# TimingSpace/MVOScaleRecovery

Hardware: AMD Instinct MI355X
Metric: frames/sec scale-recovery, KITTI-00 flow (~2k feats/frame), 1/2/4/8 GPU (higher is better)
Workload: dtype f64

## Files before the change

mvoscalerecovery_amd/csrc/mvosr_kernels.hip:

```cpp
#include <hip/hip_runtime.h>
#include <math.h>
#include <stdint.h>
#include <stdlib.h>
#include <string.h>

#include "../../include/mvosr.h"
#include "mvosr_device.hpp"
#include "mvosr_host.hpp"

namespace mvosr {

#ifdef MVOSR_STAMPS
#define MVOSR_STAMP(i) do { if (threadIdx.x == 0 && stamps) stamps[i] = __builtin_amdgcn_s_memtime(); } while (0)
#define MVOSR_STAMP_DECL unsigned long long stamps[12] = {0,0,0,0,0,0,0,0,0,0,0,0};
#define MVOSR_STAMP_ARG , unsigned long long *stamps = nullptr
#define MVOSR_STAMP_PASS , stamps
#define MVOSR_RSTAMP(i) do { if (stamps) stamps[i] = __builtin_amdgcn_s_memtime(); } while (0)
#else
#define MVOSR_RSTAMP(i) do {} while (0)
#define MVOSR_STAMP(i) do {} while (0)
#define MVOSR_STAMP_DECL
#define MVOSR_STAMP_ARG
#define MVOSR_STAMP_PASS
#endif
// ... 15 lines not shown
    p.misc = p.red + 8u * (uint32_t)(kRedSlots * 2 * waves);
    p.total = p.misc + 4u * 32u;
    return p;
}

struct Smem {
    double2 *P;
    double *Y;
    uint16_t *c16;
    uint32_t *c32;
    uint32_t *sel;
    int *hist;
    double *red;
    int *misc;
};
__device__ __forceinline__ Smem carve(char *base, int n, int waves) {
    const LdsPlan p = lds_plan(n, waves);
    Smem s;
    s.P = reinterpret_cast<double2 *>(base + p.p);
    s.Y = reinterpret_cast<double *>(base + p.y);
    s.c16 = reinterpret_cast<uint16_t *>(base + p.c);
    s.c32 = reinterpret_cast<uint32_t *>(base + p.c);
    s.sel = reinterpret_cast<uint32_t *>(base + p.c);
    s.hist = reinterpret_cast<int *>(base + p.hist);
    s.red = reinterpret_cast<double *>(base + p.red);
    s.misc = reinterpret_cast<int *>(base + p.misc);
    return s;
}

enum { M_WCNT = 0 , M_LIST = 16, M_MEDLO = 18, M_MEDHI = 20  };


constexpr int kTC = 2;


typedef double dvec2 __attribute__((ext_vector_type(2)));
__device__ __forceinline__ double2 stream_load2(const double2 *p) {
    const dvec2 v = __builtin_nontemporal_load(reinterpret_cast<const dvec2 *>(p));
    double2 r; r.x = v.x; r.y = v.y;
    return r;
}
__device__ __forceinline__ double stream_load(const double *p) {
    return __builtin_nontemporal_load(p);
}

template <int B>
struct TriChunk {
    TriIds q[kTC];
    template <bool STREAM = false>
    __device__ __forceinline__ void load(const int32_t *tri, int64_t begin, int count, int base, int tid) {
#pragma unroll
        for (int k = 0; k < kTC; ++k) {
            const int t = base + k * B + tid;
            if (t < count) {
                if constexpr (STREAM) {
                    const int32_t *p = tri + 3 * begin + 3 * t;
                    q[k].a = __builtin_nontemporal_load(p); q[k].b = __builtin_nontemporal_load(p + 1); q[k].c = __builtin_nontemporal_load(p + 2);
                } else {
                    q[k] = load_tri(tri + 3 * begin, t);
                }
            }
        }
    }
};

struct VoteFlags { bool f0, f1, f2; };
// ... 232 lines not shown
    pitch = asin(-uy) * 180.0 / 3.141592653589793;
    if (pitch < thr_deg) r |= 1;
    if (pitch >= thr_deg) r |= 2;
    return r;
}
__device__ __attribute__((noinline)) int pitch_reference_cold(double x0, double y0, double z0, double x1, double y1, double z1,
                                                              double x2, double y2, double z2, double thr_deg) {
    double nx, ny, nz, pitch;
    return pitch_reference_impl<false>(x0, y0, z0, x1, y1, z1, x2, y2, z2, thr_deg, nx, ny, nz, pitch);
}
template <bool FULL>
__device__ __forceinline__ int pitch_reference(double x0, double y0, double z0, double x1, double y1, double z1,
                                               double x2, double y2, double z2, double thr_deg,
                                               double &nx, double &ny, double &nz, double &pitch) {
    if constexpr (FULL) return pitch_reference_impl<true>(x0, y0, z0, x1, y1, z1, x2, y2, z2, thr_deg, nx, ny, nz, pitch);
    else { nx = ny = nz = pitch = 0.0; return pitch_reference_cold(x0, y0, z0, x1, y1, z1, x2, y2, z2, thr_deg); }
}

struct SelectResult {
    double height_level;
    int n_pitch, n_tri_valid;
    int singular, bad;
    int n_steep;
    int near;
};

enum { MODE_HOT = 0, MODE_EXACT = 1, MODE_FULL = 2 };

struct PitchTest {
    double thr_deg;
    double s2_hi, s2_lo;
};

template <bool FULL>
__device__ __forceinline__ int classify_triangle(double x0, double y0, double z0, double x1, double y1, double z1,
                                                 double x2, double y2, double z2, double h, const PitchTest &pt,
                                                 double *g_normals, double *g_pitch, double *g_heights, int64_t tg) {
    bool is_flat = false, is_steep = false, is_singular = false;
    bool decided = false;
    if constexpr (!FULL) {
        const double e1x = x1 - x0, e1y = y1 - y0, e1z = z1 - z0;
        const double e2x = x2 - x0, e2y = y2 - y0, e2z = z2 - z0;
        const double cx = __builtin_fma(e1y, e2z, -(e1z * e2y));
        const double cy = __builtin_fma(e1z, e2x, -(e1x * e2z));
        const double cz = __builtin_fma(e1x, e2y, -(e1y * e2x));
        const double tx = x0 * cx, ty = y0 * cy, tz = z0 * cz;
        const double det = (tx + ty) + tz;
        const double mag = (fabs(tx) + fabs(ty)) + fabs(tz);
        const double c2 = __builtin_fma(cz, cz, __builtin_fma(cy, cy, cx * cx));
        const double q2 = cy * cy;
        const double sy = cy * det;
        const bool safe = fabs(det) > 1e-9 * mag;
        is_flat = safe & (sy > 0.0) & (q2 > pt.s2_hi * c2);
        is_steep = safe & ((sy <= 0.0) | (q2 < pt.s2_lo * c2));
        decided = is_flat | is_steep;
    }
    if (!decided) {
        double nx, ny, nz, pitch;
        const int r = pitch_reference<FULL>(x0, y0, z0, x1, y1, z1, x2, y2, z2, pt.thr_deg, nx, ny, nz, pitch);
        is_singular = r & 4;
        is_flat = r & 1;
        is_steep = r & 2;
        if constexpr (FULL) {
            if (g_normals) { double *o = g_normals + 3 * tg; o[0] = nx; o[1] = ny; o[2] = nz; }
            if (g_pitch) g_pitch[tg] = pitch;
            if (g_heights) g_heights[tg] = h;
        }
    }
    return (is_flat ? 1 : 0) | (is_steep ? 2 : 0) | (is_singular ? 4 : 0) | (decided ? 0 : 8);
}

template <bool FULL, class Fetch>
struct SteepStream {
    const int32_t *tri;
    const int32_t *order;
    int t2n;
    const PitchTest &pt;
    Fetch fetch;
    int t_next;
    unsigned long long mask;
    double h;
    __device__ __forceinline__ void refill() {
        const int t = t_next + lane_id();
        bool steep = false;
        h = 0.0;
        if (t < t2n) {
            const int row = order ? min(max(order[t], 0), t2n - 1) : t;
            const TriIds q = load_tri(tri, row);
            double x0, y0, z0, x1, y1, z1, x2, y2, z2;
            if (fetch(q, x0, y0, z0, x1, y1, z1, x2, y2, z2)) {
// ... 81 lines not shown
        });
        __threadfence_block();
        __syncthreads();
        if (tid == 0) {
            double val[kNpDepth + 1];
            int vp = 0, kk = 0;
            np_pairwise_leaves(m, [&](int, int, bool is_leaf) {
                if (is_leaf) val[vp++] = leaf[kk++];
                else { const double r = val[--vp], l = val[--vp]; val[vp++] = l + r; }
            });
            *slot = c0 == 0 ? val[0] : *slot + val[0];
        }
        __syncthreads();
    }
    res = *slot;
    __syncthreads();
    return (0.0 + res) / (double)n_steep;
}

struct LdsFetch {
    const double2 *P; const double *Y; int n_valid;
    __device__ __forceinline__ bool operator()(const TriIds q, double &x0, double &y0, double &z0, double &x1, double &y1, double &z1,
                                               double &x2, double &y2, double &z2) const {
        if ((unsigned)q.a >= (unsigned)n_valid || (unsigned)q.b >= (unsigned)n_valid || (unsigned)q.c >= (unsigned)n_valid) return false;
        const double2 p0 = P[q.a], p1 = P[q.b], p2 = P[q.c];
        x0 = p0.x; z0 = p0.y; x1 = p1.x; z1 = p1.y; x2 = p2.x; z2 = p2.y;
        y0 = Y[q.a]; y1 = Y[q.b]; y2 = Y[q.c];
        return true;
    }
};

constexpr double kLevelGuard = 1e-12;

template <int WAVES, int MODE, int FW = 1>
__device__ __forceinline__ SelectResult phase_select(const Smem &s, int n_valid, const int32_t *tri2, int64_t t2_begin,
                                                     int t2_count, TriChunk<WAVES * kWave> &tc, PitchTest pt,
                                                     double *g_normals, double *g_pitch, double *g_heights, int bad_in,
                                                     double *scratch, int scratch_cap MVOSR_STAMP_ARG) {
    constexpr int B = WAVES * kWave;
    constexpr bool FULL = MODE == MODE_FULL;
    const int tid = threadIdx.x;
    unsigned long long flat = 0ull;
    unsigned long long flat_hi = 0ull;
    double hsum = 0.0, hcnt = 0.0, habs = 0.0;
    int npitch = 0, singular = 0, bad = 0;
    int undecided = 0;
    if (t2_count > 64 * FW * B) { bad = 1; t2_count = 0; }
    auto test_triangle = [&](int t, int kk, const TriIds q) {
    if ((unsigned)q.a >= (unsigned)n_valid || (unsigned)q.b >= (unsigned)n_valid || (unsigned)q.c >= (unsigned)n_valid) { bad = 1; return; }
    const double2 p0 = s.P[q.a], p1 = s.P[q.b], p2 = s.P[q.c];
    const double y0 = s.Y[q.a], y1 = s.Y[q.b], y2 = s.Y[q.c];
    const double x0 = p0.x, z0 = p0.y, x1 = p1.x, z1 = p1.y, x2 = p2.x, z2 = p2.y;
    const double h = MODE == MODE_HOT ? (y0 + y1) + y2 : div3((y0 + y1) + y2);
    const int r = classify_triangle<FULL>(x0, y0, z0, x1, y1, z1, x2, y2, z2, h, pt, g_normals, g_pitch, g_heights, t2_begin + t);
    const bool is_flat = r & 1, is_steep = r & 2;
    if (r & 4) singular = 1;
    if constexpr (MODE == MODE_HOT) { if (r & 8) undecided = 1; }
    if (is_steep) { hsum += h; hcnt += 1.0; if constexpr (MODE == MODE_HOT) habs += fabs(h); }
    if (is_flat) {
        if (FW == 1 || kk < 64) flat |= 1ull << (kk & 63); else flat_hi |= 1ull << (kk & 63);
        ++npitch;
    }
    };
    TriChunk<B> tn;
    for (int base = 0; base < t2_count; base += kTC * B) {
        const bool more = base + kTC * B < t2_count;
        if (more) tn.load(tri2, t2_begin, t2_count, base + kTC * B, tid);
#pragma unroll
        for (int k = 0; k < kTC; ++k) {
            const int t = base + k * B + tid;
            if (t < t2_count) test_triangle(t, base / B + k, tc.q[k]);
        }
        if (more) tc = tn;
    }
    const bool in_regs = t2_count <= kTC * B;
    if (!in_regs && t2_count > 0) tc.template load<true>(tri2, t2_begin, t2_count, 0, tid);
    if constexpr (MODE == MODE_HOT) block_sum3<WAVES>(hsum, hcnt, habs, s.red + R_SEL_H * 2 * WAVES, s.red + R_SEL_ABS * 2 * WAVES);
    else block_sum2<WAVES>(hsum, hcnt, s.red + R_SEL_H * 2 * WAVES);
    MVOSR_STAMP(4);
    SelectResult r;
    double hl = hsum / hcnt;
    const double guard = kLevelGuard * (habs / hcnt);
    if constexpr (MODE != MODE_HOT) {
        if (scratch && (int)hcnt + kNpMaxLeaves <= scratch_cap)
            hl = exact_height_level_block<WAVES, FULL>(tri2 + 3 * t2_begin, t2_count, (int)hcnt, pt, LdsFetch{s.P, s.Y, n_valid}, nullptr,
                                                       scratch, s.misc + M_WCNT, s.red + R_MISC * 2 * WAVES);
        else
            hl = exact_height_level<FULL>(tri2 + 3 * t2_begin, t2_count, (int)hcnt, pt, LdsFetch{s.P, s.Y, n_valid});
    }
    int ntv = 0, near = undecided;
    auto mark_triangle = [&](int kk, int qa, int qb, int qc) {
        const unsigned long long fw = (FW == 1 || kk < 64) ? flat : flat_hi;
        if (!((fw >> (kk & 63)) & 1ull)) return;
        const double y0 = s.Y[qa], y1 = s.Y[qb], y2 = s.Y[qc];
        const double h = MODE == MODE_HOT ? (y0 + y1) + y2 : div3((y0 + y1) + y2);
        if constexpr (MODE == MODE_HOT) { if (fabs(h - hl) <= guard) near = 1; }
        if (h > hl) {
            ++ntv;
            atomicOr(&s.sel[qa >> 5], 1u << (qa & 31));
            atomicOr(&s.sel[qb >> 5], 1u << (qb & 31));
            atomicOr(&s.sel[qc >> 5], 1u << (qc & 31));
        }
    };
    for (int base = 0; base < t2_count; base += kTC * B) {
        const bool more = base + kTC * B < t2_count;
        if (more) tn.template load<true>(tri2, t2_begin, t2_count, base + kTC * B, tid);
#pragma unroll
        for (int k = 0; k < kTC; ++k) {
            if (base + k * B + tid < t2_count) mark_triangle(base / B + k, tc.q[k].a, tc.q[k].b, tc.q[k].c);
        }
        if (more) tc = tn;
    }
    bad |= bad_in;
    int sn = singular | (near << 16);
    block_sum4i<WAVES>(npitch, ntv, sn, bad, s.red + R_SEL_CNT * 2 * WAVES);
    singular = sn & 0xFFFF;
    r.near = sn >> 16;
    MVOSR_STAMP(5);
    r.height_level = MODE == MODE_HOT ? hl / 3.0 : hl;
    r.n_steep = (int)hcnt;
    r.n_pitch = npitch; r.n_tri_valid = ntv; r.singular = singular; r.bad = bad;
    return r;
}

struct RoadResult {
    double height;
    int status;
    int n_sel, n_kept, n_modes, mode_left, mode_right;
    double mean, std, skew, median;
};

__device__ __forceinline__ bool dropped_by_single(double y, int bin, const Bits192 &single, int first_single) {
    bool d = false;
#pragma unroll
    for (int dk = -1; dk <= 1; ++dk) {
        const int k = bin + dk;
        const bool is_single = (k >= 0) && (k < kBins) && single.test_lane(max(k, 0));
// ... 401 lines not shown
    int32_t *c = a.o.counts + f * MVOSR_N_COUNTS;
    c[MVOSR_CNT_VALID] = nvalid; c[MVOSR_CNT_TRI_PITCH] = npitch; c[MVOSR_CNT_TRI_VALID] = ntv;
    c[MVOSR_CNT_SELECTED] = R.n_sel; c[MVOSR_CNT_KEPT] = R.n_kept; c[MVOSR_CNT_MODES] = R.n_modes;
    c[MVOSR_CNT_MODE_LEFT] = R.mode_left; c[MVOSR_CNT_MODE_RIGHT] = R.mode_right;
}

__device__ __forceinline__ bool early_frame_exit(const KArgs &a, int64_t f, int n, int t2n) {
    const bool too_few = n == 3;
    const bool oversize = n > a.b.max_feat;
    if (!(n <= 2 || too_few || t2n <= 0 || oversize)) return false;
    if (threadIdx.x == 0) {
        RoadResult R;
        R.n_sel = R.n_kept = R.n_modes = 0; R.mode_left = R.mode_right = -1;
        a.o.raw_scale[f] = nan(""); a.o.height[f] = nan(""); a.o.height_level[f] = nan("");
        a.o.status[f] = oversize ? MVOSR_ST_ERR_MASK : (too_few ? MVOSR_ST_TOO_FEW : MVOSR_ST_ERR_EMPTY);
        a.nsel[f] = 0;
        write_counts(a, f, too_few ? n : 0, 0, 0, R);
    }
    return true;
}

template <int BW, int MODE>
__device__ __forceinline__ void frame_tail(const KArgs &a, const Smem &s, int64_t f, int64_t off, int nvalid, bool refused,
                                           SelectResult &S, RoadResult &R) {
    constexpr int B = BW * kWave;
    const int tid = threadIdx.x;
    int status = kStPending;
    double raw = nan("");
    int nsel = 0;
    if (refused || S.bad) {
        status = MVOSR_ST_ERR_MASK;
    } else if (S.singular) {
        status = MVOSR_ST_ERR_SINGULAR;
    } else {
        const int w = wave_id(), lane = lane_id();
        const int per = ((nvalid + B - 1) / B) * kWave;
        const int begin = w * per, end = min(nvalid, begin + per);
        int cnt = 0;
        for (int j0 = begin; j0 < end; j0 += kWave) {
            const int j = j0 + lane;
            const bool sel = (j < end) && ((s.sel[j >> 5] >> (j & 31)) & 1u);
            if (a.o.selected && j < end) a.o.selected[off + j] = (uint8_t)sel;
            cnt += __popcll(__ballot(sel));
        }
        if (lane == 0) s.misc[M_WCNT + w] = cnt;
        __syncthreads();
        int base = 0;
#pragma unroll
        for (int i = 0; i < BW; ++i) { const int c = s.misc[M_WCNT + i]; if (i < w) base += c; nsel += c; }
        if constexpr (MODE == MODE_HOT) {
            if (S.near || nsel == 0) {
                if (tid == 0) { a.redo[1 + atomicAdd(a.redo, 1)] = (int32_t)f; a.o.status[f] = kStRedo; a.nsel[f] = 0; }
                return;
            }
        }
        double *dst = a.ysel + off;
        for (int j0 = begin; j0 < end; j0 += kWave) {
            const int j = j0 + lane;
            const bool sel = (j < end) && ((s.sel[j >> 5] >> (j & 31)) & 1u);
            const unsigned long long m = __ballot(sel);
            if (sel) dst[base + __popcll(m & ((1ull << lane) - 1ull))] = s.Y[j];
            base += __popcll(m);
        }
        if (nsel == 0) { status = MVOSR_ST_NO_FLAT; raw = a.P.absolute_reference / S.height_level; }
    }
    if (tid == 0) {
// ... 35 lines not shown
    MVOSR_STAMP_DECL
    MVOSR_STAMP(11);
    const int n = a.b.feat_cnt[f];
    const int64_t off = a.b.feat_off[f];
    const int64_t t1b = a.b.tri1_off[f], t2b = a.b.tri2_off[f];
    const int t1n = tri_rows(a.b.tri1_off, a.b.tri1_cnt, f), t2n = tri_rows(a.b.tri2_off, a.b.tri2_cnt, f);
    const Smem s = carve(smem, n, WAVES);
#ifdef MVOSR_STAMPS
    if (n < 0) return;
#endif
    MVOSR_STAMP(0);
#ifdef MVOSR_STAMPS
    if (threadIdx.x == 0) {
        stamps[10] = (unsigned long long)__builtin_amdgcn_s_getreg((31 << 11) | 4) | ((unsigned long long)__builtin_amdgcn_s_getreg((31 << 11) | 20) << 32);
    }
#endif

    RoadResult R;
    R.height = nan(""); R.n_sel = R.n_kept = R.n_modes = 0; R.mode_left = R.mode_right = -1;
    R.mean = R.std = R.skew = R.median = nan("");
    if (early_frame_exit(a, f, n, t2n)) return;
    int bad = 0;
    TriChunk<B> tc2;
    const int nvalid = phase_vote<WAVES, SC>(s, n, a.b.x + off, a.b.y + off, a.b.z + off, a.b.v + off, a.b.tri1, t1b, t1n,
                                             a.P.cos_pitch, a.P.sin_pitch,
                                             a.o.vote_counters ? a.o.vote_counters + off : nullptr, bad,
                                             a.b.tri2, t2b, t2n, tc2, a.P.vote_mode == MVOSR_VOTE_FIXED MVOSR_STAMP_PASS);
    const bool mask_mismatch = a.b.n2_expected && a.b.n2_expected[f] != nvalid;

    SelectResult S;
    S.height_level = nan(""); S.n_pitch = S.n_tri_valid = 0; S.singular = 0; S.bad = 1; S.n_steep = 0; S.near = 0;
    const bool too_many_rows = t1n > kMaxVoteRows;
    if (!mask_mismatch && !too_many_rows)
        S = phase_select<WAVES, MODE>(s, nvalid, a.b.tri2, t2b, t2n, tc2, a.pt, a.o.tri_normals, a.o.tri_pitch_deg,
                                      a.o.tri_heights, bad, a.ysel ? a.ysel + off : nullptr, n MVOSR_STAMP_PASS);
    frame_tail<WAVES, MODE>(a, s, f, off, nvalid, mask_mismatch || too_many_rows, S, R);
    MVOSR_STAMP(9);
#ifdef MVOSR_STAMPS
    if (threadIdx.x == 0 && a.o.hist) { unsigned long long *d = reinterpret_cast<unsigned long long *>(a.o.hist + f * 2 * kBins); for (int i = 0; i < 12; ++i) d[i] = stamps[i]; }
#endif
    });
}

struct DenseWs { double2 *P2; double *Y2; };

__host__ __device__ inline uint32_t dense_lds_bytes(int n, int waves) {
    const uint32_t npad = (uint32_t)((n + 1) & ~1);
    return align16(2u * npad + 16u) + align16(4u * ((uint32_t)(n + 31) / 32u)) + 8u * (uint32_t)(kRedSlots * 2 * waves) + 4u * 32u;
}

template <int DW, bool FUSED>
__device__ __forceinline__ int phase_vote_dense(uint32_t *c32, int *misc, int n, const double *gx, const double *gy, const double *gz,
                                                const double *gv, const int32_t *tri1, int64_t t1_begin, int t1_count,
                                                double cp, double sp, int32_t *g_counters, int &bad,
                                                double2 *P2, double *Y2, bool fixed) {
    constexpr int B = DW * kWave;
    const int tid = threadIdx.x, w = wave_id(), lane = lane_id();
    const uint16_t *c16 = reinterpret_cast<const uint16_t *>(c32);
    const uint32_t ones = ((uint32_t)(kCounterBias + 1) << 16) | (uint32_t)(kCounterBias + 1);
    for (int i = tid; i < ((n + 1) >> 1); i += B) c32[i] = ones;
    __threadfence_block();
    __syncthreads();
    const bool checked = t1_count > kMaxVoteRows;
    for (int t = tid; t < t1_count; t += B) {
        const TriIds q = load_tri(tri1 + 3 * t1_begin, t);
        if ((unsigned)q.a >= (unsigned)n || (unsigned)q.b >= (unsigned)n || (unsigned)q.c >= (unsigned)n) { bad = 1; continue; }
        double2 p0, p1, p2;
// ... 131 lines not shown
    const int nvalid = phase_vote_dense<DW, false>(c32, misc, n, nullptr, gy, gz, a.b.v + off, a.b.tri1, t1b, t1n, cp, sp,
                                                   a.o.vote_counters ? a.o.vote_counters + off : nullptr, bad, nullptr, nullptr,
                                                   a.P.vote_mode == MVOSR_VOTE_FIXED);
    const bool mask_mismatch = a.b.n2_expected && a.b.n2_expected[f] != nvalid;
    SelectResult S;
    S.height_level = nan(""); S.n_pitch = S.n_tri_valid = 0; S.singular = 0; S.bad = 1; S.n_steep = 0; S.near = 0;
    const int32_t *tri = a.b.tri2 + 3 * t2b;
    auto fetch = [=](const TriIds q, double &x0, double &y0, double &z0, double &x1, double &y1, double &z1,
                     double &x2, double &y2, double &z2) -> bool {
        const bool ok = (unsigned)q.a < (unsigned)n && (unsigned)q.b < (unsigned)n && (unsigned)q.c < (unsigned)n &&
                        c16[q.a] >= kCounterBias && c16[q.b] >= kCounterBias && c16[q.c] >= kCounterBias;
        if (!ok) return false;
        const double ya = gy[q.a], za = gz[q.a], yb = gy[q.b], zb = gz[q.b], yc = gy[q.c], zc = gz[q.c];
        x0 = gx[q.a]; x1 = gx[q.b]; x2 = gx[q.c];
        y0 = ya * cp - za * sp; y1 = yb * cp - zb * sp; y2 = yc * cp - zc * sp;
        z0 = ya * sp + za * cp; z1 = yb * sp + zb * cp; z2 = yc * sp + zc * cp;
        return true;
    };
    if (!mask_mismatch) {
        unsigned long long flat = 0ull, flat_hi = 0ull;
        double hsum = 0.0, hcnt = 0.0, habs = 0.0;
        int npitch = 0, singular = 0, ntv = 0, near = 0;
        if (t2n > 128 * B) bad = 1;
        const int t2s = bad ? 0 : t2n;
        TriIds cur = {0, 0, 0};
        if (tid < t2s) cur = load_tri(tri, tid);
        for (int base = 0, kk = 0; base < t2s; base += B, ++kk) {
            const TriIds q = cur;
            if (base + B + tid < t2s) cur = load_tri(tri, base + B + tid);
            if (base + tid >= t2s) continue;
            double x0, y0, z0, x1, y1, z1, x2, y2, z2;
            if (!fetch(q, x0, y0, z0, x1, y1, z1, x2, y2, z2)) { bad = 1; continue; }
            const double h = div3((y0 + y1) + y2);
            const int r = classify_triangle<FULL>(x0, y0, z0, x1, y1, z1, x2, y2, z2, h, a.pt, a.o.tri_normals, a.o.tri_pitch_deg,
                                                  a.o.tri_heights, t2b + base + tid);
            if (r & 4) singular = 1;
            if (r & 2) { hsum += h; hcnt += 1.0; if constexpr (MODE == MODE_HOT) habs += fabs(h); }
            if (r & 1) {
                if (kk < 64) flat |= 1ull << (kk & 63); else flat_hi |= 1ull << (kk & 63);
                ++npitch;
            }
        }
        cur = {0, 0, 0};
        if (tid < t2s) cur = load_tri(tri, tid);
        if constexpr (MODE == MODE_HOT) block_sum3<DW>(hsum, hcnt, habs, red + R_SEL_H * 2 * DW, red + R_SEL_ABS * 2 * DW);
        else block_sum2<DW>(hsum, hcnt, red + R_SEL_H * 2 * DW);
        double hl = hsum / hcnt;
        const double guard = kLevelGuard * (habs / hcnt);
        if constexpr (MODE != MODE_HOT)
            hl = exact_height_level<FULL>(tri, t2s, (int)hcnt, a.pt, fetch, a.b.tri2_order ? a.b.tri2_order + t2b : nullptr);
        for (int base = 0, kk = 0; base < t2s; base += B, ++kk) {
            const TriIds q = cur;
            if (base + B + tid < t2s) cur = load_tri(tri, base + B + tid);
            const unsigned long long fw = kk < 64 ? flat : flat_hi;
            if (base + tid < t2s && ((fw >> (kk & 63)) & 1ull)) {
                const double y0 = gy[q.a] * cp - gz[q.a] * sp, y1 = gy[q.b] * cp - gz[q.b] * sp, y2 = gy[q.c] * cp - gz[q.c] * sp;
                const double h = div3((y0 + y1) + y2);
                if constexpr (MODE == MODE_HOT) { if (fabs(h - hl) <= guard) near = 1; }
                if (h > hl) {
                    ++ntv;
                    atomicOr(&sel[q.a >> 5], 1u << (q.a & 31));
                    atomicOr(&sel[q.b >> 5], 1u << (q.b & 31));
                    atomicOr(&sel[q.c >> 5], 1u << (q.c & 31));
                }
            }
        }
        int sn = singular | (near << 16);
        block_sum4i<DW>(npitch, ntv, sn, bad, red + R_SEL_CNT * 2 * DW);
        S.height_level = hl; S.n_steep = (int)hcnt; S.near = sn >> 16;
        S.n_pitch = npitch; S.n_tri_valid = ntv; S.singular = sn & 0xFFFF; S.bad = bad;
    }
    int status = kStPending;
    double raw = nan("");
    int nsel = 0;
    if (mask_mismatch || S.bad) {
        status = MVOSR_ST_ERR_MASK;
    } else if (S.singular) {
        status = MVOSR_ST_ERR_SINGULAR;
    } else {
        const int per = ((n + B - 1) / B) * kWave;
        const int begin = w * per, end = min(n, begin + per);
        int nv = 0, ns = 0;
        for (int i0 = begin; i0 < end; i0 += kWave) {
            const int i = i0 + lane;
            const bool valid = (i < end) && c16[i] >= kCounterBias;
            const bool on = valid && ((sel[i >> 5] >> (i & 31)) & 1u);
            nv += __popcll(__ballot(valid));
            ns += __popcll(__ballot(on));
        }
        if (lane == 0) { misc[M_WCNT + w] = ns; misc[M_WCNT + DW + w] = nv; }
        __syncthreads();
        int base_s = 0, base_v = 0;
#pragma unroll
        for (int i = 0; i < DW; ++i) { const int c = misc[M_WCNT + i]; if (i < w) { base_s += c; base_v += misc[M_WCNT + DW + i]; } nsel += c; }
        if constexpr (MODE == MODE_HOT) {
            if (S.near || nsel == 0) {
                if (tid == 0) { a.redo[1 + atomicAdd(a.redo, 1)] = (int32_t)f; a.o.status[f] = kStRedo; a.nsel[f] = 0; }
                return;
            }
        }
        double *dst = a.ysel + off;
        for (int i0 = begin; i0 < end; i0 += kWave) {
            const int i = i0 + lane;
            const bool valid = (i < end) && c16[i] >= kCounterBias;
            const bool on = valid && ((sel[i >> 5] >> (i & 31)) & 1u);
            const unsigned long long mv = __ballot(valid), ms = __ballot(on);
            const unsigned long long below = (1ull << lane) - 1ull;
            if (valid && a.o.selected) a.o.selected[off + base_v + __popcll(mv & below)] = (uint8_t)on;
            if (on) dst[base_s + __popcll(ms & below)] = gy[i] * cp - gz[i] * sp;
            base_v += __popcll(mv);
            base_s += __popcll(ms);
// ... 117 lines not shown
#pragma unroll
        for (int j = 0; j < VPT; ++j) {
            if (j * B + tid >= W) continue;
            const int i = t * W + j * B + tid, slot = sb + j * B + tid;
            double2 pa, pb;
            pa.x = tv[j]; pa.y = ty[j] * sp + tz[j] * cp;
            pb.x = tx[j]; pb.y = ty[j] * cp - tz[j] * sp;
            if (i < n) { ringA[slot] = pa; ringB[slot] = pb; }
            ringC[slot] = 1;
            ringH[slot] = 0ull;
            used[slot] = 0;
        }
    };
    tile_load(0); tile_store(0);
    tile_load(1); tile_store(1);
    tile_load(2);
    {
        int b0 = bad, b1 = 0, b2 = 0, b3 = 0;
        block_sum4i<DW>(b0, b1, b2, b3, red + R_MISC * 2 * DW);
        bad = b0;
    }
    if (bad) {
        if (tid == 0) {
            a.o.raw_scale[f] = nan(""); a.o.height[f] = nan(""); a.o.height_level[f] = nan("");
            a.o.status[f] = MVOSR_ST_ERR_MASK; a.nsel[f] = 0;
            write_counts(a, f, 0, 0, 0, R);
        }
        return;
    }
    MVOSR_TSTAMP(0);

    double hsum = 0.0, hcnt = 0.0;
    bool sneg = false, spos = false, mixed_signs = false;
    int npitch = 0, singular = 0, nvalid = 0, overflow = 0;
    const int rid = tid;

    const int far1 = toff1[ntiles], far2 = toff2[ntiles];
    const double *fart = nullptr;
    if (a.b.tile_far && a.b.tile_far_off) {
        const int64_t fb = a.b.tile_far_off[f];
        if (a.b.tile_far_off[f + 1] - fb != 9 * ((int64_t)(t1n - far1) + (int64_t)(t2n - far2))) bad = 1;
        else fart = a.b.tile_far + fb;
    }
    for (int t = far1 + tid; t < t1n; t += B) {
        const TriIds q = load_tri(rows1, t);
        if ((unsigned)q.a >= (unsigned)n || (unsigned)q.b >= (unsigned)n || (unsigned)q.c >= (unsigned)n) { bad = 1; continue; }
        double2 p0, p1, p2;
        if (fart) {
            const double *r = fart + 9 * (t - far1);
            p0.x = r[2]; p0.y = r[0] * sp + r[1] * cp;
            p1.x = r[5]; p1.y = r[3] * sp + r[4] * cp;
            p2.x = r[8]; p2.y = r[6] * sp + r[7] * cp;
        } else {
            p0.x = gv[q.a]; p0.y = gy[q.a] * sp + gz[q.a] * cp;
            p1.x = gv[q.b]; p1.y = gy[q.b] * sp + gz[q.b] * cp;
            p2.x = gv[q.c]; p2.y = gy[q.c] * sp + gz[q.c] * cp;
        }
        const bool pa = (p0.x - p1.x) * (p0.y - p1.y) > 0.0;
        const bool pb = (p0.x - p2.x) * (p0.y - p2.y) > 0.0;
        const bool pc = (p1.x - p2.x) * (p1.y - p2.y) > 0.0;
        const int e = atomicAdd(n_pendV, 3);
        if (e + 3 <= kPendCap) {
            const VoteFlags vf = vote_flags(pa, pb, pc, fixed);
            pendV[e] = q.a << 1 | (vf.f0 ? 1 : 0);
            pendV[e + 1] = q.b << 1 | (vf.f1 ? 1 : 0);
            pendV[e + 2] = q.c << 1 | (vf.f2 ? 1 : 0);
        } else overflow = 1;
    }
    for (int t = far2 + tid; t < t2n; t += B) {
        const TriIds q = load_tri(rows2, t);
        if ((unsigned)q.a >= (unsigned)n || (unsigned)q.b >= (unsigned)n || (unsigned)q.c >= (unsigned)n) { bad = 1; continue; }
        double xa, ya, za, xb, yb, zb, xc, yc, zc;
        if (fart) {
            const double *r = fart + 9 * ((t1n - far1) + (t - far2));
            xa = r[0]; ya = r[1]; za = r[2]; xb = r[3]; yb = r[4]; zb = r[5]; xc = r[6]; yc = r[7]; zc = r[8];
        } else {
            xa = gx[q.a]; ya = gy[q.a]; za = gz[q.a]; xb = gx[q.b]; yb = gy[q.b]; zb = gz[q.b]; xc = gx[q.c]; yc = gy[q.c]; zc = gz[q.c];
        }
        const double y0 = ya * cp - za * sp, y1 = yb * cp - zb * sp, y2 = yc * cp - zc * sp;
        const double h = (y0 + y1) + y2;
        const int r = classify_triangle<false>(xa, y0, ya * sp + za * cp, xb, y1, yb * sp + zb * cp,
                                               xc, y2, yc * sp + zc * cp, h, a.pt, nullptr, nullptr, nullptr, 0);
        if (r & 4) singular = 1;
        if (r & 2) { hsum += h; hcnt += 1.0; sneg |= h < 0.0; spos |= h > 0.0; }
        if (r & 1) ++npitch;
        const unsigned long long key = ((r & 1) && h == h) ? height_key64(h) : 0ull;
        const int e = atomicAdd(n_pendH, 3);
        if (e + 3 <= kPendCapH) {
            pendH[e] = key; pendH[e + 1] = key; pendH[e + 2] = key;
            pendHv[e] = q.a; pendHv[e + 1] = q.b; pendHv[e + 2] = q.c;
        } else overflow = 1;
    }
    __syncthreads();
    auto apply_pending = [&](int tile) {
        const int nv = min(n_pendV[0], kPendCap), nh = min(n_pendH[0], kPendCapH), sb = tile_slot(tile);
        for (int e = tid; e < nv; e += B) {
            const int p = pendV[e], vtx = p >> 1;
            if (vtx / W == tile) atomicAdd(&ringC[sb + vtx - tile * W], (p & 1) ? -1 : 1);
        }
        for (int e = tid; e < nh; e += B) {
            const int vtx = pendHv[e];
            if (vtx / W == tile) { const unsigned long long key = pendH[e]; if (key) atomicMax(&ringH[sb + vtx - tile * W], key); used[sb + vtx - tile * W] = 1; }
        }
    };
    apply_pending(0);
    MVOSR_TSTAMP(1);

    const int32_t *rows1c = t1n > 0 ? rows1 : rows2;
    TriIds n1[kTileRows], n2[kTileRows];
    auto prefetch_rows = [&](int k) {
        const int last1 = max(min(toff1[k + 1], max(t1n, 1)) - 1, 0), last2 = max(min(toff2[k + 1], t2n) - 1, 0);
#pragma unroll
        for (int j = 0; j < kTileRows; ++j) {
            n1[j] = load_tri(rows1c, min(toff1[k] + j * B + rid, last1));
            n2[j] = load_tri(rows2, min(toff2[k] + j * B + rid, last2));
        }
// ... 56 lines not shown
        {
            double2 vp[kTileRows][3];
            bool ok[kTileRows];
#pragma unroll
            for (int j = 0; j < kTileRows; ++j) {
                const TriIds q = c1[j];
                const bool live = b1 + j * B + rid < e1;
                ok[j] = live && row_ok(q);
                if (live && !ok[j]) bad = 1;
                if (ok[j]) { vp[j][0] = ringA[S(q.a)]; vp[j][1] = ringA[S(q.b)]; vp[j][2] = ringA[S(q.c)]; }
            }
#pragma unroll
            for (int j = 0; j < kTileRows; ++j) {
                if (!ok[j]) continue;
                const TriIds q = c1[j];
                const double2 p0 = vp[j][0], p1 = vp[j][1], p2 = vp[j][2];
                const bool pa = (p0.x - p1.x) * (p0.y - p1.y) > 0.0;
                const bool pb = (p0.x - p2.x) * (p0.y - p2.y) > 0.0;
                const bool pc = (p1.x - p2.x) * (p1.y - p2.y) > 0.0;
                const VoteFlags vf = vote_flags(pa, pb, pc, fixed);
                atomicAdd(&ringC[S(q.a)], vf.f0 ? -1 : 1);
                atomicAdd(&ringC[S(q.b)], vf.f1 ? -1 : 1);
                atomicAdd(&ringC[S(q.c)], vf.f2 ? -1 : 1);
            }
        }
        for (int t = b1 + kTileRows * B + rid; t < e1; t += B) vote_row(load_tri(rows1, t));
        MVOSR_TSTAMP(2);
        auto select_row = [&](const TriIds q) {
            if (!row_ok(q)) { bad = 1; return; }
            const double2 a0 = ringA[S(q.a)], a1 = ringA[S(q.b)], a2 = ringA[S(q.c)];
            const double2 g0_ = ringB[S(q.a)], g1_ = ringB[S(q.b)], g2_ = ringB[S(q.c)];
            used[S(q.a)] = 1; used[S(q.b)] = 1; used[S(q.c)] = 1;
            const double h = (g0_.y + g1_.y) + g2_.y;
            const int r = classify_triangle<false>(g0_.x, g0_.y, a0.y, g1_.x, g1_.y, a1.y, g2_.x, g2_.y, a2.y, h, a.pt,
                                                   nullptr, nullptr, nullptr, 0);
            if (r & 4) singular = 1;
            if (r & 2) { hsum += h; hcnt += 1.0; sneg |= h < 0.0; spos |= h > 0.0; }
            if (r & 1) {
                ++npitch;
                if (h == h) {
                    const unsigned long long key = height_key64(h);
                    atomicMax(&ringH[S(q.a)], key); atomicMax(&ringH[S(q.b)], key); atomicMax(&ringH[S(q.c)], key);
                }
            }
        };
#pragma unroll
        for (int j = 0; j < kTileRows; ++j) { if (b2 + j * B + rid < e2) select_row(c2[j]); }
        for (int t = b2 + kTileRows * B + rid; t < e2; t += B) select_row(load_tri(rows2, t));
        MVOSR_TSTAMP(3);
        if (k > 0) retire(k - 1);
        tile_store(k + 2);
        tile_load(k + 3);
        MVOSR_TSTAMP(5);
        __syncthreads();
        MVOSR_TSTAMP(6);
    }
    retire(ntiles - 1);

    block_sum2<DW>(hsum, hcnt, red + R_SEL_H * 2 * DW);
    {
        const int wf = (__ballot(singular != 0) ? 1 : 0) | (__ballot(bad != 0) ? 1 << 8 : 0) | (__ballot(overflow != 0) ? 1 << 16 : 0);
        int sb = (lane == 0) ? wf : 0;
        int nv = (lane == 0) ? nvalid : 0;
        int z0 = (lane == 0) ? ((__ballot(sneg) ? 1 : 0) | (__ballot(spos) ? 1 << 8 : 0)) : 0;
        block_sum4i<DW>(npitch, nv, sb, z0, red + R_SEL_CNT * 2 * DW);
        nvalid = nv; singular = sb & 0xFF; bad = (sb >> 8) & 0xFF; overflow = sb >> 16;
        mixed_signs = (z0 & 0xFF) && (z0 >> 8);
    }
    MVOSR_TSTAMP(7);
    const double hl = hsum / hcnt;
    const bool mask_mismatch = a.b.n2_expected && a.b.n2_expected[f] != nvalid;
    int status = kStPending;
    double raw = nan("");
    int nsel = 0;
    if (overflow && !bad) {
        if (tid == 0) { a.redo[1 + atomicAdd(a.redo, 1)] = (int32_t)f; a.o.status[f] = kStRedo; a.nsel[f] = 0; }
        return;
    }
    if (mask_mismatch || bad) {
        status = MVOSR_ST_ERR_MASK;
    } else if (singular) {
        status = MVOSR_ST_ERR_SINGULAR;
    } else {
        constexpr int kTailBatch = 8;
        const int nchunks = (cand_cnt + 63) >> 6;
        const double *my_h = cand_h + cand_base, *my_y = cand_y + cand_base;
        unsigned long long selbits = 0ull;
        int cnt = 0, near = (hl == hl && !mixed_signs) ? 0 : 1;
        for (int cb = 0; cb < nchunks; cb += kTailBatch) {
            double hm[kTailBatch];
#pragma unroll
            for (int j = 0; j < kTailBatch; ++j) hm[j] = my_h[min(((cb + j) << 6) + lane, max(cand_cnt, 1) - 1)];
#pragma unroll
            for (int j = 0; j < kTailBatch; ++j) {
                const bool have = ((cb + j) << 6) + lane < cand_cnt;
                if (have && fabs(hm[j] - hl) <= kLevelGuard * fabs(hl)) near = 1;
                const bool sel = have && hm[j] > hl;
                if (sel && cb + j < 64) selbits |= 1ull << (cb + j);
                cnt += __popcll(__ballot(sel));
            }
        }
        const int wave_near = __ballot(near != 0) != 0ull;
        if (lane == 0) { misc[M_WCNT + w] = cnt; misc[M_WCNT + DW + w] = wave_near; }
        __syncthreads();
        int base = 0, any_near = 0;
#pragma unroll
        for (int i = 0; i < DW; ++i) { const int c = misc[M_WCNT + i]; if (i < w) base += c; nsel += c; any_near |= misc[M_WCNT + DW + i]; }
        MVOSR_TSTAMP(8);
        if (any_near || nsel == 0) {
            if (tid == 0) { a.redo[1 + atomicAdd(a.redo, 1)] = (int32_t)f; a.o.status[f] = kStRedo; a.nsel[f] = 0; }
            return;
        }
        double *dst = a.ysel + off;
        for (int cb = 0; cb < nchunks; cb += kTailBatch) {
            double yv[kTailBatch], hm[kTailBatch];
#pragma unroll
            for (int j = 0; j < kTailBatch; ++j) {
                const int at = min(((cb + j) << 6) + lane, max(cand_cnt, 1) - 1);
                yv[j] = my_y[at];
                hm[j] = nchunks > 64 ? my_h[at] : 0.0;
            }
// ... 650 lines not shown
```

Baseline: 26.31 million.

## Skip exact pitch fallback in hot path and cache flat heights across sweeps

In the hot mode, the classifier no longer falls back to the exact pitch reference for undecided triangles. Undecided triangles are instead flagged, and the flag pushes the frame onto the existing near/exact redo path, replacing the singular-status handling in the fused kernels. The hot select also keeps the flat-triangle heights for the first four chunks in registers, so the second selection sweep can reuse them instead of recomputing geometry. This trades extra register pressure and a more complex control flow for less divergent fallback work and less recomputation.

```diff
diff --git a/mvoscalerecovery_amd/csrc/mvosr_kernels.hip b/mvoscalerecovery_amd/csrc/mvosr_kernels.hip
--- a/mvoscalerecovery_amd/csrc/mvosr_kernels.hip
+++ b/mvoscalerecovery_amd/csrc/mvosr_kernels.hip
@@ -71,6 +71,7 @@
 
 
 constexpr int kTC = 2;
+constexpr int kKeepRows = 4 * kTC;
 
 
 typedef double dvec2 __attribute__((ext_vector_type(2)));
@@ -369,7 +370,7 @@
     double s2_hi, s2_lo;
 };
 
-template <bool FULL>
+template <bool FULL, bool HOT = false>
 __device__ __forceinline__ int classify_triangle(double x0, double y0, double z0, double x1, double y1, double z1,
                                                  double x2, double y2, double z2, double h, const PitchTest &pt,
                                                  double *g_normals, double *g_pitch, double *g_heights, int64_t tg) {
@@ -392,7 +393,7 @@
         is_steep = safe & ((sy <= 0.0) | (q2 < pt.s2_lo * c2));
         decided = is_flat | is_steep;
     }
-    if (!decided) {
+    if (!HOT && !decided) {
         double nx, ny, nz, pitch;
         const int r = pitch_reference<FULL>(x0, y0, z0, x1, y1, z1, x2, y2, z2, pt.thr_deg, nx, ny, nz, pitch);
         is_singular = r & 4;
@@ -540,7 +541,9 @@
 
 constexpr double kLevelGuard = 1e-12;
 
-template <int WAVES, int MODE, int FW = 1>
+template <int I> struct ChunkSlot { static constexpr int value = I; };
+
+template <int WAVES, int MODE, int FW = 1, int HC = 0>
 __device__ __forceinline__ SelectResult phase_select(const Smem &s, int n_valid, const int32_t *tri2, int64_t t2_begin,
                                                      int t2_count, TriChunk<WAVES * kWave> &tc, PitchTest pt,
                                                      double *g_normals, double *g_pitch, double *g_heights, int bad_in,
@@ -554,13 +557,17 @@
     int npitch = 0, singular = 0, bad = 0;
     int undecided = 0;
     if (t2_count > 64 * FW * B) { bad = 1; t2_count = 0; }
-    auto test_triangle = [&](int t, int kk, const TriIds q) {
-    if ((unsigned)q.a >= (unsigned)n_valid || (unsigned)q.b >= (unsigned)n_valid || (unsigned)q.c >= (unsigned)n_valid) { bad = 1; return; }
+    const double not_flat = -__builtin_inf();
+    double hkeep[HC > 0 ? HC : 1];
+#pragma unroll
+    for (int i = 0; i < (HC > 0 ? HC : 1); ++i) hkeep[i] = not_flat;
+    auto test_triangle = [&](int t, int kk, const TriIds q) -> double {
+    if ((unsigned)q.a >= (unsigned)n_valid || (unsigned)q.b >= (unsigned)n_valid || (unsigned)q.c >= (unsigned)n_valid) { bad = 1; return not_flat; }
     const double2 p0 = s.P[q.a], p1 = s.P[q.b], p2 = s.P[q.c];
     const double y0 = s.Y[q.a], y1 = s.Y[q.b], y2 = s.Y[q.c];
     const double x0 = p0.x, z0 = p0.y, x1 = p1.x, z1 = p1.y, x2 = p2.x, z2 = p2.y;
     const double h = MODE == MODE_HOT ? (y0 + y1) + y2 : div3((y0 + y1) + y2);
-    const int r = classify_triangle<FULL>(x0, y0, z0, x1, y1, z1, x2, y2, z2, h, pt, g_normals, g_pitch, g_heights, t2_begin + t);
+    const int r = classify_triangle<FULL, MODE == MODE_HOT>(x0, y0, z0, x1, y1, z1, x2, y2, z2, h, pt, g_normals, g_pitch, g_heights, t2_begin + t);
     const bool is_flat = r & 1, is_steep = r & 2;
     if (r & 4) singular = 1;
     if constexpr (MODE == MODE_HOT) { if (r & 8) undecided = 1; }
@@ -569,9 +576,29 @@
         if (FW == 1 || kk < 64) flat |= 1ull << (kk & 63); else flat_hi |= 1ull << (kk & 63);
         ++npitch;
     }
+    return is_flat ? h : not_flat;
     };
     TriChunk<B> tn;
-    for (int base = 0; base < t2_count; base += kTC * B) {
+    auto sweep1 = [&](int base, auto slot) {
+        const bool more = base + kTC * B < t2_count;
+        if (more) tn.load(tri2, t2_begin, t2_count, base + kTC * B, tid);
+#pragma unroll
+        for (int k = 0; k < kTC; ++k) {
+            const int t = base + k * B + tid;
+            double hf = not_flat;
+            if (t < t2_count) hf = test_triangle(t, base / B + k, tc.q[k]);
+            if constexpr (decltype(slot)::value >= 0) hkeep[decltype(slot)::value * kTC + k] = hf;
+        }
+        if (more) tc = tn;
+    };
+    if constexpr (HC > 0) {
+        static_assert(HC == 4 * kTC && MODE == MODE_HOT, "four chunks kept");
+        if (0 * kTC * B < t2_count) sweep1(0 * kTC * B, ChunkSlot<0>{});
+        if (1 * kTC * B < t2_count) sweep1(1 * kTC * B, ChunkSlot<1>{});
+        if (2 * kTC * B < t2_count) sweep1(2 * kTC * B, ChunkSlot<2>{});
+        if (3 * kTC * B < t2_count) sweep1(3 * kTC * B, ChunkSlot<3>{});
+    }
+    for (int base = HC * B; base < t2_count; base += kTC * B) {
         const bool more = base + kTC * B < t2_count;
         if (more) tn.load(tri2, t2_begin, t2_count, base + kTC * B, tid);
 #pragma unroll
@@ -610,7 +637,30 @@
             atomicOr(&s.sel[qc >> 5], 1u << (qc & 31));
         }
     };
-    for (int base = 0; base < t2_count; base += kTC * B) {
+    auto sweep2 = [&](int base, auto slot) {
+        const bool more = base + kTC * B < t2_count;
+        if (more) tn.template load<true>(tri2, t2_begin, t2_count, base + kTC * B, tid);
+#pragma unroll
+        for (int k = 0; k < kTC; ++k) {
+            const double h = hkeep[decltype(slot)::value * kTC + k];
+            const TriIds q = tc.q[k];
+            if (fabs(h - hl) <= guard) near = 1;
+            if (h > hl) {
+                ++ntv;
+                atomicOr(&s.sel[q.a >> 5], 1u << (q.a & 31));
+                atomicOr(&s.sel[q.b >> 5], 1u << (q.b & 31));
+                atomicOr(&s.sel[q.c >> 5], 1u << (q.c & 31));
+            }
+        }
+        if (more) tc = tn;
+    };
+    if constexpr (HC > 0) {
+        if (0 * kTC * B < t2_count) sweep2(0 * kTC * B, ChunkSlot<0>{});
+        if (1 * kTC * B < t2_count) sweep2(1 * kTC * B, ChunkSlot<1>{});
+        if (2 * kTC * B < t2_count) sweep2(2 * kTC * B, ChunkSlot<2>{});
+        if (3 * kTC * B < t2_count) sweep2(3 * kTC * B, ChunkSlot<3>{});
+    }
+    for (int base = HC * B; base < t2_count; base += kTC * B) {
         const bool more = base + kTC * B < t2_count;
         if (more) tn.template load<true>(tri2, t2_begin, t2_count, base + kTC * B, tid);
 #pragma unroll
@@ -1078,6 +1128,7 @@
         status = MVOSR_ST_ERR_MASK;
     } else if (S.singular) {
         status = MVOSR_ST_ERR_SINGULAR;
+        S.height_level = nan("");
     } else {
         const int w = wave_id(), lane = lane_id();
         const int per = ((nvalid + B - 1) / B) * kWave;
@@ -1179,7 +1230,7 @@
     S.height_level = nan(""); S.n_pitch = S.n_tri_valid = 0; S.singular = 0; S.bad = 1; S.n_steep = 0; S.near = 0;
     const bool too_many_rows = t1n > kMaxVoteRows;
     if (!mask_mismatch && !too_many_rows)
-        S = phase_select<WAVES, MODE>(s, nvalid, a.b.tri2, t2b, t2n, tc2, a.pt, a.o.tri_normals, a.o.tri_pitch_deg,
+        S = phase_select<WAVES, MODE, 1, (MODE == MODE_HOT && SC == 4) ? kKeepRows : 0>(s, nvalid, a.b.tri2, t2b, t2n, tc2, a.pt, a.o.tri_normals, a.o.tri_pitch_deg,
                                       a.o.tri_heights, bad, a.ysel ? a.ysel + off : nullptr, n MVOSR_STAMP_PASS);
     frame_tail<WAVES, MODE>(a, s, f, off, nvalid, mask_mismatch || too_many_rows, S, R);
     MVOSR_STAMP(9);
@@ -1377,9 +1428,10 @@
             double x0, y0, z0, x1, y1, z1, x2, y2, z2;
             if (!fetch(q, x0, y0, z0, x1, y1, z1, x2, y2, z2)) { bad = 1; continue; }
             const double h = div3((y0 + y1) + y2);
-            const int r = classify_triangle<FULL>(x0, y0, z0, x1, y1, z1, x2, y2, z2, h, a.pt, a.o.tri_normals, a.o.tri_pitch_deg,
-                                                  a.o.tri_heights, t2b + base + tid);
+            const int r = classify_triangle<FULL, MODE == MODE_HOT>(x0, y0, z0, x1, y1, z1, x2, y2, z2, h, a.pt, a.o.tri_normals, a.o.tri_pitch_deg,
+                                                                    a.o.tri_heights, t2b + base + tid);
             if (r & 4) singular = 1;
+            if constexpr (MODE == MODE_HOT) { if (r & 8) near = 1; }
             if (r & 2) { hsum += h; hcnt += 1.0; if constexpr (MODE == MODE_HOT) habs += fabs(h); }
             if (r & 1) {
                 if (kk < 64) flat |= 1ull << (kk & 63); else flat_hi |= 1ull << (kk & 63);
@@ -1422,6 +1474,7 @@
         status = MVOSR_ST_ERR_MASK;
     } else if (S.singular) {
         status = MVOSR_ST_ERR_SINGULAR;
+        S.height_level = nan("");
     } else {
         const int per = ((n + B - 1) / B) * kWave;
         const int begin = w * per, end = min(n, begin + per);
@@ -1605,7 +1658,7 @@
 
     double hsum = 0.0, hcnt = 0.0;
     bool sneg = false, spos = false, mixed_signs = false;
-    int npitch = 0, singular = 0, nvalid = 0, overflow = 0;
+    int npitch = 0, undecided = 0, nvalid = 0, overflow = 0;
     const int rid = tid;
 
     const int far1 = toff1[ntiles], far2 = toff2[ntiles];
@@ -1652,9 +1705,9 @@
         }
         const double y0 = ya * cp - za * sp, y1 = yb * cp - zb * sp, y2 = yc * cp - zc * sp;
         const double h = (y0 + y1) + y2;
-        const int r = classify_triangle<false>(xa, y0, ya * sp + za * cp, xb, y1, yb * sp + zb * cp,
-                                               xc, y2, yc * sp + zc * cp, h, a.pt, nullptr, nullptr, nullptr, 0);
-        if (r & 4) singular = 1;
+        const int r = classify_triangle<false, true>(xa, y0, ya * sp + za * cp, xb, y1, yb * sp + zb * cp,
+                                                     xc, y2, yc * sp + zc * cp, h, a.pt, nullptr, nullptr, nullptr, 0);
+        if (r & 8) undecided = 1;
         if (r & 2) { hsum += h; hcnt += 1.0; sneg |= h < 0.0; spos |= h > 0.0; }
         if (r & 1) ++npitch;
         const unsigned long long key = ((r & 1) && h == h) ? height_key64(h) : 0ull;
@@ -1777,9 +1830,9 @@
             const double2 g0_ = ringB[S(q.a)], g1_ = ringB[S(q.b)], g2_ = ringB[S(q.c)];
             used[S(q.a)] = 1; used[S(q.b)] = 1; used[S(q.c)] = 1;
             const double h = (g0_.y + g1_.y) + g2_.y;
-            const int r = classify_triangle<false>(g0_.x, g0_.y, a0.y, g1_.x, g1_.y, a1.y, g2_.x, g2_.y, a2.y, h, a.pt,
-                                                   nullptr, nullptr, nullptr, 0);
-            if (r & 4) singular = 1;
+            const int r = classify_triangle<false, true>(g0_.x, g0_.y, a0.y, g1_.x, g1_.y, a1.y, g2_.x, g2_.y, a2.y, h, a.pt,
+                                                         nullptr, nullptr, nullptr, 0);
+            if (r & 8) undecided = 1;
             if (r & 2) { hsum += h; hcnt += 1.0; sneg |= h < 0.0; spos |= h > 0.0; }
             if (r & 1) {
                 ++npitch;
@@ -1804,12 +1857,12 @@
 
     block_sum2<DW>(hsum, hcnt, red + R_SEL_H * 2 * DW);
     {
-        const int wf = (__ballot(singular != 0) ? 1 : 0) | (__ballot(bad != 0) ? 1 << 8 : 0) | (__ballot(overflow != 0) ? 1 << 16 : 0);
+        const int wf = (__ballot(undecided != 0) ? 1 : 0) | (__ballot(bad != 0) ? 1 << 8 : 0) | (__ballot(overflow != 0) ? 1 << 16 : 0);
         int sb = (lane == 0) ? wf : 0;
         int nv = (lane == 0) ? nvalid : 0;
         int z0 = (lane == 0) ? ((__ballot(sneg) ? 1 : 0) | (__ballot(spos) ? 1 << 8 : 0)) : 0;
         block_sum4i<DW>(npitch, nv, sb, z0, red + R_SEL_CNT * 2 * DW);
-        nvalid = nv; singular = sb & 0xFF; bad = (sb >> 8) & 0xFF; overflow = sb >> 16;
+        nvalid = nv; undecided = sb & 0xFF; bad = (sb >> 8) & 0xFF; overflow = sb >> 16;
         mixed_signs = (z0 & 0xFF) && (z0 >> 8);
     }
     MVOSR_TSTAMP(7);
@@ -1824,14 +1877,12 @@
     }
     if (mask_mismatch || bad) {
         status = MVOSR_ST_ERR_MASK;
-    } else if (singular) {
-        status = MVOSR_ST_ERR_SINGULAR;
     } else {
         constexpr int kTailBatch = 8;
         const int nchunks = (cand_cnt + 63) >> 6;
         const double *my_h = cand_h + cand_base, *my_y = cand_y + cand_base;
         unsigned long long selbits = 0ull;
-        int cnt = 0, near = (hl == hl && !mixed_signs) ? 0 : 1;
+        int cnt = 0, near = (hl == hl && !mixed_signs && !undecided) ? 0 : 1;
         for (int cb = 0; cb < nchunks; cb += kTailBatch) {
             double hm[kTailBatch];
 #pragma unroll
```

Result: no change. 26.26 million (median of 2 runs) (-0.2%).
